# SidRama/Longitudinal-VAE

Hardware: AMD Instinct MI355X
Metric: ELBO-steps/sec (exact-KL L-VAE step, Health-MNIST N=4096 L=16) (higher is better)
Workload: dtype f16x3-split (fp32-equivalent)

## Files before the change

longitudinal-vae_amd/csrc/kl_hyper.hip:

```cpp
#include "blkinv.hpp"
#include "gram_tab.hpp"
#include "prof.hpp"

namespace lvae {

constexpr int kHbMaxBin = 4;
constexpr int kHbBins = 128;
constexpr int kHbBins2 = 4096;
constexpr int kHbRun = 64;
constexpr int kHbSmall = 16;
constexpr int kHbSmallest = 4;
constexpr int kHbNear = 4;
constexpr int kHbBlk = 4;
constexpr int kHbT = 64;
constexpr int kHbTP = 68;
constexpr int kHbNB = 24;
constexpr int kHbNQ = kHbNB / 4;
constexpr int kHbNearS = 2 * kHbBins2;
constexpr int kHbNearK = kHbNearS + kHbNear + 1;
constexpr int kHbA = kHbNearK + kHbNear;
constexpr int kHbTail = 2 * kHbNear + 1 + kHbBins;
constexpr int kHbPart = 2 * kHbBins2 + kHbTail;

struct HbDev {
  int on, nbin, big, nbins, nb2, nnear;
  int gmin[kTabMaxBits], grng[kTabMaxBits];
  int wmin[kTabMaxG], wrng[kTabMaxG];
  int bmask[kHbMaxBin], bgrp[kHbMaxBin], boff[kHbMaxBin], bn[kHbMaxBin], b2off[kHbMaxBin];
  int cbin[LVAE_MAX_COMP];
  int nslot[kHbNear];
};

typedef unsigned hb_u32x4 __attribute__((ext_vector_type(4)));

struct HbWs {
  HbDev* dev;
  uint8_t* pbin;
  int* rs;
  int* re;
  double* part;
  float* tab;
  hb_u32x4* rkey;
  double* hscr;
  double* nscr;
  size_t bytes;
  HbWs(char* base, int np_, int L) {
    size_t off = 0;
    auto take = [&](size_t b) {
      char* p = base ? base + off : nullptr;
      off += align256(b);
      return p;
    };
    dev = (HbDev*)take(sizeof(HbDev));
    pbin = (uint8_t*)take((size_t)kHbMaxBin * np_);
    rs = (int*)take((size_t)np_ * sizeof(int));
    re = (int*)take((size_t)np_ * sizeof(int));
    part = (double*)take((size_t)L * (np_ / kHbT) * kHbPart * sizeof(double));
    tab = (float*)take((size_t)L * kTabMaxBwdLds * sizeof(float));
    rkey = (hb_u32x4*)take((size_t)np_ * sizeof(hb_u32x4));
    hscr = (double*)take((size_t)L * (np_ / kHbT) * kHbBins * kHbT * sizeof(double));
    nscr = (double*)take((size_t)L * (np_ / kHbT) * kHbNB * 256 * sizeof(double));
    bytes = off;
  }
};
size_t kl_hyper_bytes(int np_, int L) { return HbWs(nullptr, np_, L).bytes; }
HbDev* kl_hyper_dev(void* base, int np_, int L) { return HbWs((char*)base, np_, L).dev; }

__global__ __launch_bounds__(1024) void hb_plan_kernel(GramTab tb, const double* __restrict__ x, int ldx, int n,
                                                       int np_, const int* __restrict__ covflag, HbWs ws, int enable) {
  __shared__ int lo[kTabMaxBits + kTabMaxG], hi[kTabMaxBits + kTabMaxG];
  __shared__ int fail;
  __shared__ HbDev d;
  const int tid = threadIdx.x, nd = tb.nbits + tb.ng;
  if (*covflag != 2) {
    if (tid == 0) ws.dev->on = 0;
    return;
  }
  if (tid < kTabMaxBits + kTabMaxG) {
    lo[tid] = INT_MAX;
    hi[tid] = INT_MIN;
  }
  if (tid == 0) fail = 0;
  __syncthreads();
  for (int q = 0; q < nd; ++q) {
    const int dim = q < tb.nbits ? tb.bdim[q] : tb.gdim[q - tb.nbits];
    if (dim < 0) continue;
    int mn = INT_MAX, mx = INT_MIN;
    for (int i = tid; i < n; i += 1024) {
      const int v = (int)x[(int64_t)i * ldx + dim];
      mn = min(mn, v);
      mx = max(mx, v);
    }
#pragma unroll
    for (int o = 32; o > 0; o >>= 1) {
      mn = min(mn, __shfl_xor(mn, o, 64));
      mx = max(mx, __shfl_xor(mx, o, 64));
    }
    if ((tid & 63) == 0) {
      atomicMin(&lo[q], mn);
      atomicMax(&hi[q], mx);
    }
  }
  __syncthreads();
  if (tid == 0) {
    HbDev p{};
    int f = 0;
    p.big = -1;
    for (int b = 0; b < tb.nbits; ++b) {
      p.gmin[b] = lo[b];
      p.grng[b] = hi[b] - lo[b] + 1;
      if (tb.bkind[b] == LVAE_CAT && p.grng[b] > kHbSmallest && (p.big < 0 || p.grng[b] > p.grng[p.big])) p.big = b;
    }
    for (int b = 0; b < tb.nbits; ++b)
      if (b != p.big && tb.bkind[b] == LVAE_CAT && p.grng[b] > kHbSmall) f = 1;
    for (int g = 0; g < tb.ng; ++g) {
      p.wmin[g] = tb.gdim[g] >= 0 ? lo[tb.nbits + g] : 0;
      p.wrng[g] = tb.gdim[g] >= 0 ? hi[tb.nbits + g] - lo[tb.nbits + g] + 1 : 1;
    }
    for (int r = 0; r < tb.n_comp; ++r) {
      p.cbin[r] = -1;
      if (p.big >= 0 && ((tb.cmask[r] >> p.big) & 1)) continue;
      const int grp = tb.ckind[r] >= 0 ? tb.cgrp[r] : -1;
      int g = 0;
      while (g < p.nbin && !(p.bmask[g] == tb.cmask[r] && p.bgrp[g] == grp)) ++g;
      if (g == p.nbin) {
        if (p.nbin == kHbMaxBin) {
          f = 1;
          break;
        }
        long long nb = grp >= 0 ? p.wrng[grp] : 1;
        for (int b = 0; b < tb.nbits; ++b)
          if ((tb.cmask[r] >> b) & 1) nb *= p.grng[b];
        if (nb > kHbBins) {
          f = 1;
          break;
        }
        p.bmask[g] = tb.cmask[r];
        p.bgrp[g] = grp;
        p.bn[g] = (int)nb;
        p.boff[g] = p.nbins;
        p.b2off[g] = p.nb2;
        p.nbins += (int)nb;
        p.nb2 += (int)(nb * nb);
        ++p.nbin;
      }
      p.cbin[r] = g;
    }
    if (p.nbins > kHbBins || p.nb2 > kHbBins2) f = 1;
    {
      int nblk = 0;
      for (int g = 0; g < p.nbin; ++g) nblk += (p.bn[g] + 31) / 32;
      if (nblk > kHbBlk) f = 1;
    }
    for (int k = 0; k < tb.pbeg[tb.ng] && !f; ++k)
      if (p.cbin[tb.pcomp[tb.porder[k]]] < 0) {
        if (p.nnear == kHbNear) f = 1;
        else p.nslot[p.nnear++] = k;
      }
    d = p;
    fail = f;
  }
  __syncthreads();
  const int bd = d.big >= 0 ? tb.bdim[d.big] : -1;
  int bad = 0;
  for (int i = tid; i < np_; i += 1024) {
    int s = -1, e = -1;
    if (bd >= 0 && i < n) {
      const double v = x[(int64_t)i * ldx + bd];
      if (i > 0 && x[(int64_t)(i - 1) * ldx + bd] > v) bad = 1;
      s = i;
      while (s > 0 && i - s < kHbRun && x[(int64_t)(s - 1) * ldx + bd] == v) --s;
      e = i + 1;
      while (e < n && e - i < kHbRun && x[(int64_t)e * ldx + bd] == v) ++e;
      if (e - s > kHbRun || (s > 0 && x[(int64_t)(s - 1) * ldx + bd] == v) || (e < n && x[(int64_t)e * ldx + bd] == v))
        bad = 1;
    }
    ws.rs[i] = s;
    ws.re[i] = e;
    hb_u32x4 key = {0u, 0u, 0u, 0u};
    if (i < n) {
      for (int b = 0; b < tb.nbits; ++b) {
        const int xv = (int)x[(int64_t)i * ldx + tb.bdim[b]], v = xv - d.gmin[b];
        if (b == d.big) continue;
        if (tb.bkind[b] == LVAE_CAT) {
          if (v < 0 || v > 63) bad = 1;
          key.x |= (unsigned)(v & 63) << (6 * b);
        } else {
          if (xv != 0 && xv != 1) bad = 1;
          key.w |= (unsigned)(xv == 1) << b;
        }
      }
      for (int g = 0; g < tb.ng; ++g) {
        if (tb.gdim[g] < 0) continue;
        const int v = (int)x[(int64_t)i * ldx + tb.gdim[g]] - d.wmin[g];
        if (v < 0 || v > 65535) bad = 1;
        const unsigned u = (unsigned)(v & 0xffff);
        if (g == 0) key.y |= u;
        else if (g == 1) key.y |= u << 16;
        else key.z |= u;
      }
    }
    ws.rkey[i] = key;
    for (int g = 0; g < kHbMaxBin; ++g) {
      int idx = 255;
      if (g < d.nbin && i < n) {
        idx = 0;
        for (int b = 0; b < tb.nbits; ++b)
          if ((d.bmask[g] >> b) & 1) idx = idx * d.grng[b] + ((int)x[(int64_t)i * ldx + tb.bdim[b]] - d.gmin[b]);
        if (d.bgrp[g] >= 0) idx = idx * d.wrng[d.bgrp[g]] + ((int)x[(int64_t)i * ldx + tb.gdim[d.bgrp[g]]] - d.wmin[d.bgrp[g]]);
      }
      ws.pbin[(size_t)g * np_ + i] = (uint8_t)idx;
    }
  }
  if (__any(bad) && (tid & 63) == 0) atomicOr(&fail, 1);
  __syncthreads();
  if (tid == 0) {
    HbDev p = d;
    p.on = (!fail && enable) ? 1 : 0;
    *ws.dev = p;
  }
}


__global__ __launch_bounds__(256) void hb_tab_kernel(GramTab tb, HbWs ws, const double* __restrict__ params) {
  __shared__ float sp[64];
  const int tid = threadIdx.x, l = blockIdx.y, e = blockIdx.x * 256 + tid;
  if (!ws.dev->on) return;
  if (tid < tb.n_params) sp[tid] = float(params[(int64_t)l * tb.n_params + tid]);
  __syncthreads();
  if (e < tb.pbeg[tb.ng] * (1 << tb.nbits) * kTabR) ws.tab[(int64_t)l * kTabMaxBwdLds + e] = tab_bwd_entry(tb, sp, e);
}

__device__ inline unsigned hb_pair_code(hb_u32x4 ki, hb_u32x4 kj, unsigned catbits, int ng) {
  const unsigned x = ki.x ^ kj.x, x1 = x | (x >> 1), x3 = x1 | (x1 >> 2), x5 = x3 | (x1 >> 4);
  const unsigned fail = (((x5 & 0x1041041u) * 0x108421u) >> 20) & 31u;
  unsigned c = (catbits & ~fail) | (ki.w & kj.w);
  const unsigned a0 = ki.y & 0xffffu, b0 = kj.y & 0xffffu, a1 = ki.y >> 16, b1 = kj.y >> 16;
  const unsigned a2 = ki.z & 0xffffu, b2 = kj.z & 0xffffu;
  const unsigned d0 = a0 > b0 ? a0 - b0 : b0 - a0, d1 = a1 > b1 ? a1 - b1 : b1 - a1, d2 = a2 > b2 ? a2 - b2 : b2 - a2;
  const unsigned cap = (unsigned)kTabD;
  c |= (d0 < cap ? d0 : cap) << 8;
  if (ng > 1) c |= (d1 < cap ? d1 : cap) << 16;
  if (ng > 2) c |= (d2 < cap ? d2 : cap) << 24;
  return c;
}

__device__ inline unsigned hb_catbits(const GramTab& tb) {
  unsigned m = 0;
#pragma unroll
  for (int b = 0; b < kTabMaxBits; ++b)
    if (b < tb.nbits && tb.bkind[b] == LVAE_CAT) m |= 1u << b;
  return m;
}

__device__ inline void hb_near_tables(const GramTab& tb, const HbDev& d, const float* __restrict__ gt, int tstride,
                                      float* __restrict__ tab, int* __restrict__ sgrp) {
  const int tid = threadIdx.x;
  if (tid < d.nnear) sgrp[tid] = tb.cgrp[tb.pcomp[tb.porder[d.nslot[tid]]]];
  for (int e = tid; e < d.nnear * tstride; e += blockDim.x) tab[e] = gt[d.nslot[e / tstride] * tstride + e % tstride];
}

__device__ inline float hb_near_d(const float* tab, int tk, unsigned code, int grp) {
  return tab[tk + (int)(code & 0xffu) * kTabR + (int)((code >> (8 * (grp + 1))) & 0xffu)];
}

__global__ __launch_bounds__(256) void hb_near_kernel(GramTab tb, HbWs ws, int n, int np_,
                                                      const float* __restrict__ Kinv, const double* __restrict__ alpha) {
  __shared__ HbDev d;
  __shared__ int sgrp[kHbNear];
  __shared__ double red[4][kHbNear];
  extern __shared__ float ntab[];
  const int tid = threadIdx.x, lane = tid & 63, w = tid >> 6, I = blockIdx.x, l = blockIdx.y, I0 = I * kHbT;
  if (tid == 0) d = *ws.dev;
  __syncthreads();
  if (!d.on) return;
  const int tstride = (1 << tb.nbits) * kTabR, nnear = d.nnear;
  hb_near_tables(tb, d, ws.tab + (int64_t)l * kTabMaxBwdLds, tstride, ntab, sgrp);
  __syncthreads();
  const float* K = Kinv + (int64_t)l * np_ * np_;
  const double* al = alpha + (int64_t)l * np_;
  const unsigned catbits = hb_catbits(tb);
  double acc[kHbNear];
#pragma unroll
  for (int k = 0; k < kHbNear; ++k) acc[k] = 0.0;
  if (d.big >= 0) {
    for (int e = tid; e < kHbT * kHbRun; e += 256) {
      const int i = I0 + e / kHbRun, jj = e % kHbRun;
      if (i >= n) continue;
      const int s = ws.rs[i], len = ws.re[i] - s;
      if (jj >= len) continue;
      const int j = s + jj;
      const unsigned c = hb_pair_code(ws.rkey[i], ws.rkey[j], catbits, tb.ng);
      const double val = 0.5 * ((double)K[(int64_t)i * np_ + j] - al[i] * al[j]);
#pragma unroll
      for (int k = 0; k < kHbNear; ++k)
        if (k < nnear) acc[k] += val * (double)hb_near_d(ntab, k * tstride, c, sgrp[k]);
    }
  }
#pragma unroll
  for (int k = 0; k < kHbNear; ++k) {
    const double sk = wave_sum(acc[k]);
    if (lane == 0) red[w][k] = sk;
  }
  __syncthreads();
  if (tid < kHbNear)
    ws.part[((int64_t)l * (np_ / kHbT) + I) * kHbPart + kHbNearK + tid] =
        ((red[0][tid] + red[1][tid]) + red[2][tid]) + red[3][tid];
}


#ifdef LVAE_HB_STAMP
#define HB_STAMP(t)                                                                   \
  do {                                                                                \
    __builtin_amdgcn_sched_barrier(0);                                                \
    asm volatile("s_memtime %0\n\ts_waitcnt lgkmcnt(0)" : "=s"(t)::"memory");       \
    __builtin_amdgcn_sched_barrier(0);                                                \
  } while (0)
#else
#define HB_STAMP(t) \
  do {              \
  } while (0)
#endif

typedef float hb_f32x2 __attribute__((ext_vector_type(2)));
typedef float hb_f32x4 __attribute__((ext_vector_type(4)));
typedef float hb_f32x16 __attribute__((ext_vector_type(16)));
typedef __bf16 hb_bf16x8 __attribute__((ext_vector_type(8)));
typedef __bf16 hb_bf16x2 __attribute__((ext_vector_type(2)));
constexpr int kHbSlabThreads = 256, kHbSlabWaves = kHbSlabThreads / 64;
#ifndef LVAE_HB_FOLD
#define LVAE_HB_FOLD 16
#endif
constexpr int kHbFold = LVAE_HB_FOLD;
#ifndef LVAE_HB_DEPTH
#define LVAE_HB_DEPTH 1
#endif
constexpr int kHbDepth = LVAE_HB_DEPTH;
static_assert(kHbDepth == 1 || kHbDepth == 2 || kHbDepth == 4, "nt = np / 64 is a multiple of 4");

struct HbPre {
  hb_f32x2 pk[8];
  int pbn;
  hb_f32x4 vr[2];
};

__device__ inline unsigned hb_pk_bf16(float a, float b) {
  const hb_bf16x2 v = {(__bf16)a, (__bf16)b};
  return __builtin_bit_cast(unsigned, v);
}
__device__ inline float hb_bf_lo(unsigned u) { return __uint_as_float(u << 16); }
__device__ inline float hb_bf_hi(unsigned u) { return __uint_as_float(u & 0xffff0000u); }

__device__ inline int hb_pl_off(int c, int k) { return c * 32 + ((k ^ ((c >> 1) & 7)) << 2); }

__device__ inline void hb_split8(const float* a, hb_u32x4& hi, hb_u32x4& mid, hb_u32x4& lo) {
#pragma unroll
  for (int k = 0; k < 4; ++k) {
    const float x0 = a[2 * k], x1 = a[2 * k + 1];
    const unsigned h = hb_pk_bf16(x0, x1);
    const float r0 = x0 - hb_bf_lo(h), r1 = x1 - hb_bf_hi(h);
    const unsigned m = hb_pk_bf16(r0, r1);
    const float s0 = r0 - hb_bf_lo(m), s1 = r1 - hb_bf_hi(m);
    hi[k] = h;
    mid[k] = m;
    lo[k] = hb_pk_bf16(s0, s1);
  }
}

__global__ __launch_bounds__(kHbSlabThreads, 2) void hb_slab_kernel(GramTab tb, HbWs ws, int n, int np_,
                                                                    const float* __restrict__ Kinv,
                                                                    const float* __restrict__ vv,
                                                                    const double* __restrict__ alpha) {
  __shared__ HbDev d;
  __shared__ __attribute__((aligned(16))) float Tc[2 * kHbT * kHbTP];
  __shared__ __attribute__((aligned(16))) unsigned Pw[3][kHbT * 32];
  __shared__ __attribute__((aligned(8))) uint8_t rbin[kHbMaxBin][kHbT];
  __shared__ uint8_t cbin[kHbMaxBin][kHbT];
  __shared__ float vs[kHbT];
  __shared__ double acol[kHbT];
  __shared__ hb_u32x4 ckey[2 * kHbT];
  __shared__ int rstart[kHbT];
  __shared__ unsigned long long runends;
  __shared__ int nblk, nspan;
  __shared__ uint8_t blist[kHbNB];
  __shared__ int8_t blkid[64];
  __shared__ int sgrp[kHbNear];
  __shared__ int sbg[kHbBlk], sbb[kHbBlk], nbk;
  __shared__ double red[kHbSlabWaves][kHbNear + 1];
  extern __shared__ float tab[];
  const int tid = threadIdx.x, lane = tid & 63, w = tid >> 6, J = blockIdx.x, l = blockIdx.y, J0 = J * kHbT;
  if (tid == 0) d = *ws.dev;
  __syncthreads();
  if (!d.on) return;
  const int tstride = (1 << tb.nbits) * kTabR;
  if (tid < kHbT) {
    vs[tid] = vv[(int64_t)l * np_ + J0 + tid];
    acol[tid] = alpha[(int64_t)l * np_ + J0 + tid];
  }
  for (int e = tid; e < d.nbin * kHbT; e += kHbSlabThreads)
    cbin[e / kHbT][e % kHbT] = ws.pbin[(size_t)(e / kHbT) * np_ + J0 + e % kHbT];
  hb_near_tables(tb, d, ws.tab + (int64_t)l * kTabMaxBwdLds, tstride, tab, sgrp);
  if (tid < 2 * kHbT) {
    const int c = J0 - kHbT + tid;
    ckey[tid] = c >= 0 ? ws.rkey[c] : hb_u32x4{0u, 0u, 0u, 0u};
  }
  if (w == 0) {
    const int c = J0 + lane;
    const bool isend = d.big >= 0 && c < n && ws.re[c] == c + 1;
    const int s0 = isend ? ws.rs[c] : c;
    rstart[lane] = s0;
    const int ba = (s0 - J0 + kHbT) >> 4, bz = (c - J0 + kHbT) >> 4;
    unsigned long long m = 0;
    if (isend)
      for (int bi = ba; bi <= bz; ++bi)
        for (int bj = ba; bj <= bi; ++bj) m |= 1ull << (bi * 8 + bj);
#pragma unroll
    for (int o = 32; o > 0; o >>= 1) {
      const unsigned lo = __shfl_xor((unsigned)m, o, 64), hi = __shfl_xor((unsigned)(m >> 32), o, 64);
      m |= ((unsigned long long)hi << 32) | lo;
    }
    const unsigned long long ends = __ballot(isend), sp = __ballot(isend && s0 < J0);
    if (lane == 0) {
      runends = ends;
      nspan = sp != 0;
      int t = 0;
      for (int b = 0; b < 64; ++b) {
        blkid[b] = -1;
        if (((m >> b) & 1ull) && t < kHbNB) {
          blkid[b] = (int8_t)t;
          blist[t++] = (uint8_t)b;
        }
      }
      nblk = t;
    }
  }
  if (tid == 0) {
    int t = 0;
    for (int g = 0; g < d.nbin; ++g)
      for (int bb = 0; bb * 32 < d.bn[g] && t < kHbBlk; ++bb, ++t) {
        sbg[t] = g;
        sbb[t] = bb;
      }
    nbk = t;
  }
  __syncthreads();
  const float* K = Kinv + (int64_t)l * np_ * np_;
  const int nbin = d.nbin, nnear = d.nnear, nitem = 2 * nbk, nbl = nblk, span = nspan;
  const unsigned catbits = hb_catbits(tb);
  const int cb = w & 1, hh = lane >> 5, col = 32 * cb + (lane & 31);
  const int i0 = w, i1 = w + kHbSlabWaves;
  const bool it0 = i0 < nitem, it1 = i1 < nitem;
  int g0 = 0, b00 = 0, g1 = 0, b01 = 0;
  if (it0) {
    g0 = sbg[i0 >> 1];
    b00 = 32 * sbb[i0 >> 1];
  }
  if (it1) {
    g1 = sbg[i1 >> 1];
    b01 = 32 * sbb[i1 >> 1];
  }
  hb_f32x16 acc0 = {}, acc1 = {};
  double* Hs = ws.hscr + ((int64_t)l * (np_ / kHbT) + J) * kHbBins * kHbT;
  double* Ns = ws.nscr + ((int64_t)l * (np_ / kHbT) + J) * kHbNB * 256;
  const int li = lane & 15, lk = lane >> 4;
  bi_f32x4 nac[kHbNQ];
#pragma unroll
  for (int q = 0; q < kHbNQ; ++q) nac[q] = bi_f32x4{0.f, 0.f, 0.f, 0.f};
  double tS = 0.0;
  const int cp = tid & 31, i8 = tid >> 5;
  const float v0 = vs[2 * cp], v1 = vs[2 * cp + 1], r0 = sqrtf(v0), r1 = sqrtf(v1);
  const int nt = np_ / kHbT;

  auto fetch = [&](int I, HbPre& p) {
    const int I0 = I * kHbT;
#pragma unroll
    for (int u = 0; u < 8; ++u)
      p.pk[u] = __builtin_nontemporal_load(
          reinterpret_cast<const hb_f32x2*>(K + (int64_t)(I0 + 8 * i8 + u) * np_ + J0 + 2 * cp));
    p.pbn = (int)ws.pbin[(size_t)(w < nbin ? w : 0) * np_ + I0 + lane];
    const float* vr = vv + (int64_t)l * np_ + I0 + 8 * i8;
    p.vr[0] = *reinterpret_cast<const hb_f32x4*>(vr);
    p.vr[1] = *reinterpret_cast<const hb_f32x4*>(vr + 4);
  };

  auto fold = [&](hb_f32x16& acc, int g, int b0, bool first) {
    const int nb = d.bn[g];
    double* hc = Hs + (int64_t)d.boff[g] * kHbT + col;
#pragma unroll
    for (int e = 0; e < 16; ++e) {
      const int b = b0 + (e & 3) + 8 * (e >> 2) + 4 * hh;
      if (b < nb) {
        if (first) hc[b * kHbT] = (double)acc[e];
        else unsafeAtomicAdd(hc + b * kHbT, (double)acc[e]);
      }
      acc[e] = 0.f;
    }
  };

  auto body = [&](int I, HbPre& p) {
    const int I0 = I * kHbT;
    const bool fold_now = (I & (kHbFold - 1)) == kHbFold - 1 || I == nt - 1, fold_first = I < kHbFold;
    {
      float ts = 0.f;
#pragma unroll
      for (int u = 0; u < 8; ++u) {
        const float s0 = p.pk[u][0] * r0, s1 = p.pk[u][1] * r1;
        ts += s0 * s0 + s1 * s1;
      }
      tS += (double)ts;
#pragma unroll
      for (int c = 0; c < 2; ++c) {
        float a[8];
#pragma unroll
        for (int u = 0; u < 8; ++u) a[u] = p.pk[u][c];
        hb_u32x4 hi, mid, lo;
        hb_split8(a, hi, mid, lo);
        const int off = hb_pl_off(2 * cp + c, i8);
        *reinterpret_cast<hb_u32x4*>(&Pw[0][off]) = hi;
        *reinterpret_cast<hb_u32x4*>(&Pw[1][off]) = mid;
        *reinterpret_cast<hb_u32x4*>(&Pw[2][off]) = lo;
      }
    }
    if (w < nbin) rbin[w][lane] = (uint8_t)p.pbn;
    if (nbl > 0) {
      float sr[8];
#pragma unroll
      for (int u = 0; u < 8; ++u) sr[u] = sqrtf(p.vr[u >> 2][u & 3]);
#pragma unroll
      for (int c = 0; c < 2; ++c) {
        float* dst = &Tc[(kHbT + 2 * cp + c) * kHbTP + 8 * i8];
        *reinterpret_cast<hb_f32x4*>(dst) = hb_f32x4{p.pk[0][c] * sr[0], p.pk[1][c] * sr[1], p.pk[2][c] * sr[2],
                                                     p.pk[3][c] * sr[3]};
        *reinterpret_cast<hb_f32x4*>(dst + 4) = hb_f32x4{p.pk[4][c] * sr[4], p.pk[5][c] * sr[5],
                                                         p.pk[6][c] * sr[6], p.pk[7][c] * sr[7]};
      }
      if (span) {
        hb_f32x2 q[8];
#pragma unroll
        for (int u = 0; u < 8; ++u)
          q[u] = *reinterpret_cast<const hb_f32x2*>(K + (int64_t)(I0 + 8 * i8 + u) * np_ + J0 - kHbT + 2 * cp);
#pragma unroll
        for (int c = 0; c < 2; ++c) {
          float* dst = &Tc[(2 * cp + c) * kHbTP + 8 * i8];
          *reinterpret_cast<hb_f32x4*>(dst) = hb_f32x4{q[0][c] * sr[0], q[1][c] * sr[1], q[2][c] * sr[2],
                                                       q[3][c] * sr[3]};
          *reinterpret_cast<hb_f32x4*>(dst + 4) = hb_f32x4{q[4][c] * sr[4], q[5][c] * sr[5], q[6][c] * sr[6],
                                                           q[7][c] * sr[7]};
        }
      }
    }
    __syncthreads();
    fetch(I + kHbDepth < nt ? I + kHbDepth : nt - 1, p);
    if (it0) {
      auto onehot = [&](int g, int b0, int ks) {
        const unsigned mybin = (unsigned)(b0 + (lane & 31));
        const uint2 rb = *reinterpret_cast<const uint2*>(&rbin[g][16 * ks + 8 * hh]);
        hb_u32x4 a;
#pragma unroll
        for (int k = 0; k < 4; ++k) {
          const unsigned wd = k < 2 ? rb.x : rb.y, sh = 16 * (k & 1);
          const unsigned lo_ = ((wd >> sh) & 0xffu) == mybin ? 0x3f80u : 0u;
          const unsigned hi_ = ((wd >> (sh + 8)) & 0xffu) == mybin ? 0x3f800000u : 0u;
          a[k] = lo_ | hi_;
        }
        return __builtin_bit_cast(hb_bf16x8, a);
      };
#pragma unroll
      for (int ks = 0; ks < 4; ++ks) {
        const hb_bf16x8 bh = *reinterpret_cast<const hb_bf16x8*>(&Pw[0][hb_pl_off(col, 2 * ks + hh)]);
        const hb_bf16x8 bm = *reinterpret_cast<const hb_bf16x8*>(&Pw[1][hb_pl_off(col, 2 * ks + hh)]);
        const hb_bf16x8 bl = *reinterpret_cast<const hb_bf16x8*>(&Pw[2][hb_pl_off(col, 2 * ks + hh)]);
        const hb_bf16x8 a0 = onehot(g0, b00, ks);
        acc0 = __builtin_amdgcn_mfma_f32_32x32x16_bf16(a0, bl, acc0, 0, 0, 0);
        acc0 = __builtin_amdgcn_mfma_f32_32x32x16_bf16(a0, bm, acc0, 0, 0, 0);
        acc0 = __builtin_amdgcn_mfma_f32_32x32x16_bf16(a0, bh, acc0, 0, 0, 0);
        if (it1) {
          const hb_bf16x8 a1 = onehot(g1, b01, ks);
          acc1 = __builtin_amdgcn_mfma_f32_32x32x16_bf16(a1, bl, acc1, 0, 0, 0);
          acc1 = __builtin_amdgcn_mfma_f32_32x32x16_bf16(a1, bm, acc1, 0, 0, 0);
          acc1 = __builtin_amdgcn_mfma_f32_32x32x16_bf16(a1, bh, acc1, 0, 0, 0);
        }
      }
      if (fold_now) {
        fold(acc0, g0, b00, fold_first);
        if (it1) fold(acc1, g1, b01, fold_first);
      }
    }
#pragma unroll
    for (int q = 0; q < kHbNQ; ++q) {
      const int t = w + kHbSlabWaves * q;
      if (t < nbl) {
        const int bb = blist[t], bi = bb >> 3, bj = bb & 7;
        const float* pa = &Tc[(16 * bi + li) * kHbTP + 16 * lk];
        const float* pb = &Tc[(16 * bj + li) * kHbTP + 16 * lk];
        hb_f32x4 a4[4], b4[4];
#pragma unroll
        for (int s4 = 0; s4 < 4; ++s4) {
          a4[s4] = *reinterpret_cast<const hb_f32x4*>(pa + 4 * s4);
          b4[s4] = *reinterpret_cast<const hb_f32x4*>(pb + 4 * s4);
        }
        bi_f32x4 x0 = {0.f, 0.f, 0.f, 0.f}, x1 = {0.f, 0.f, 0.f, 0.f};
#pragma unroll
        for (int s4 = 0; s4 < 4; ++s4) {
          x0 = __builtin_amdgcn_mfma_f32_16x16x4f32(a4[s4][0], b4[s4][0], x0, 0, 0, 0);
          x1 = __builtin_amdgcn_mfma_f32_16x16x4f32(a4[s4][1], b4[s4][1], x1, 0, 0, 0);
          x0 = __builtin_amdgcn_mfma_f32_16x16x4f32(a4[s4][2], b4[s4][2], x0, 0, 0, 0);
          x1 = __builtin_amdgcn_mfma_f32_16x16x4f32(a4[s4][3], b4[s4][3], x1, 0, 0, 0);
        }
        nac[q] += x0 + x1;
        if (fold_now) {
          double* nb = Ns + t * 256 + (4 * lk) * 16 + li;
#pragma unroll
          for (int e = 0; e < 4; ++e) {
            if (fold_first) nb[e * 16] = (double)nac[q][e];
            else unsafeAtomicAdd(nb + e * 16, (double)nac[q][e]);
          }
          nac[q] = bi_f32x4{0.f, 0.f, 0.f, 0.f};
        }
      }
    }
    __syncthreads();
  };

  HbPre pre[kHbDepth];
#pragma unroll
  for (int u = 0; u < kHbDepth; ++u) fetch(u, pre[u]);
  for (int I = 0; I < nt; I += kHbDepth) {
#pragma unroll
    for (int u = 0; u < kHbDepth; ++u) body(I + u, pre[u]);
  }
  __builtin_amdgcn_s_waitcnt(0);
  __threadfence_block();
  __syncthreads();
  double* Qs = reinterpret_cast<double*>(&Tc[0]);
  for (int e = tid; e < d.nb2; e += kHbSlabThreads) Qs[e] = 0.0;
  __syncthreads();
  double* out = ws.part + ((int64_t)l * nt + J) * kHbPart;
  for (int tb2 = tid; tb2 < d.nbins; tb2 += kHbSlabThreads) {
    int g = 0;
    while (g + 1 < nbin && tb2 >= d.boff[g + 1]) ++g;
    const int b = tb2 - d.boff[g], nb = d.bn[g];
    double* qrow = Qs + d.b2off[g] + b * nb;
    const double* hr = Hs + (int64_t)tb2 * kHbT;
    double as = 0.0;
    for (int m = 0; m < kHbT; ++m) {
      const int bc = cbin[g][m];
      if (bc != 255) qrow[bc] += hr[m];
      if (bc == b) as += acol[m];
    }
    out[kHbA + tb2] = as;
  }
  __syncthreads();
  for (int e = tid; e < d.nb2; e += kHbSlabThreads) out[kHbBins2 + e] = Qs[e];
  for (int g = 0; g < nbin; ++g) {
    const int nb = d.bn[g], nb16 = (nb + 15) >> 4;
    for (int item = w; item < nb16 * nb16; item += kHbSlabWaves) {
      const int bi = item / nb16, bj = item % nb16, li = lane & 15, lk = lane >> 4;
      const int ba = 16 * bi + li, bb = 16 * bj + li;
      const double* ha = Hs + (int64_t)(d.boff[g] + (ba < nb ? ba : 0)) * kHbT;
      const double* hb = Hs + (int64_t)(d.boff[g] + (bb < nb ? bb : 0)) * kHbT;
      bi_f64x4 acc = {0.0, 0.0, 0.0, 0.0};
#pragma unroll 4
      for (int s4 = 0; s4 < kHbT; s4 += 4) {
        const int m = s4 + lk;
        const double a = ba < nb ? ha[m] * (double)vs[m] : 0.0;
        const double b = bb < nb ? hb[m] : 0.0;
        acc = __builtin_amdgcn_mfma_f64_16x16x4f64(a, b, acc, 0, 0, 0);
      }
#pragma unroll
      for (int q = 0; q < 4; ++q) {
        const int r = 16 * bi + lk + 4 * q, c = 16 * bj + li;
        if (r < nb && c < nb) out[d.b2off[g] + r * nb + c] = acc[q];
      }
    }
  }
  double nacc[kHbNear];
#pragma unroll
  for (int k = 0; k < kHbNear; ++k) nacc[k] = 0.0;
  for (unsigned long long rm = runends; rm; rm &= rm - 1) {
    const int e = __builtin_ctzll(rm), s0 = rstart[e], len = e + 1 - (s0 - J0);
    for (int pq = tid; pq < len * len; pq += kHbSlabThreads) {
      const int wi = s0 - J0 + kHbT + pq / len, wj = s0 - J0 + kHbT + pq % len;
      const int lo_ = min(wi, wj), hi_ = max(wi, wj);
      const int t = blkid[((hi_ >> 4) << 3) | (lo_ >> 4)];
      const double sv = t >= 0 ? Ns[t * 256 + (hi_ & 15) * 16 + (lo_ & 15)] : 0.0;
      const unsigned c = hb_pair_code(ckey[wi], ckey[wj], catbits, tb.ng);
      const int cb8 = (int)(c & 0xffu) * kTabR;
#pragma unroll
      for (int k2 = 0; k2 < kHbNear; ++k2) {
        if (k2 >= nnear) break;
        const int g = sgrp[k2];
        nacc[k2] += sv * (double)tab[k2 * tstride + cb8 + (int)((c >> (8 * (g + 1))) & 0xffu)];
      }
    }
  }
#pragma unroll
  for (int k = 0; k < kHbNear; ++k) {
    const double sk = wave_sum(nacc[k]);
    if (lane == 0) red[w][k] = sk;
  }
  {
    const double st = wave_sum(tS);
    if (lane == 0) red[w][kHbNear] = st;
  }
  __syncthreads();
  if (tid <= kHbNear) {
    double t = 0.0;
#pragma unroll
    for (int u = 0; u < kHbSlabWaves; ++u) t += red[u][tid];
    out[kHbNearS + tid] = t;
  }
}

constexpr int kNoiseSlotHb = 64, kBwdSlotsHb = 65;

__global__ __launch_bounds__(256) void hb_sum_kernel(HbWs ws, int np_) {
  const int i = blockIdx.x * 256 + threadIdx.x, l = blockIdx.y, nt = np_ / kHbT, nb2 = ws.dev->nb2;
  if (!ws.dev->on || i >= 2 * nb2 + kHbTail) return;
  const int e = i < nb2 ? i : i < 2 * nb2 ? kHbBins2 + i - nb2 : 2 * kHbBins2 + i - 2 * nb2;
  double* pl = ws.part + (int64_t)l * nt * kHbPart + e;
  double s = 0.0;
#pragma unroll 16
  for (int J = 0; J < nt; ++J) s += pl[(int64_t)J * kHbPart];
  pl[0] = s;
}

__global__ __launch_bounds__(256) void hb_final_kernel(GramTab tb, HbWs ws, int n, int np_,
                                                       const double* __restrict__ alpha,
                                                       const double* __restrict__ kdiag, double* __restrict__ part,
                                                       int G) {
  __shared__ HbDev d;
  __shared__ double Gb[kHbBins2];
  __shared__ double raw[kBwdSlotsHb];
  __shared__ double red[4];
  __shared__ double nz;
  extern __shared__ float ftab[];
  const int tid = threadIdx.x, lane = tid & 63, w = tid >> 6, l = blockIdx.x, nt = np_ / kHbT;
  if (tid == 0) d = *ws.dev;
  __syncthreads();
  if (!d.on) return;
  if (tid < kBwdSlotsHb) raw[tid] = 0.0;
  const double* al = alpha + (int64_t)l * np_;
  const double* pl = ws.part + (int64_t)l * nt * kHbPart;
  {
    const float* gt = ws.tab + (int64_t)l * kTabMaxBwdLds;
    for (int e = tid; e < tb.pbeg[tb.ng] * (1 << tb.nbits) * kTabR; e += 256) ftab[e] = gt[e];
  }
  for (int e = tid; e < d.nb2; e += 256) {
    int g = 0;
    while (g + 1 < d.nbin && e >= d.b2off[g + 1]) ++g;
    const int nb = d.bn[g], b = (e - d.b2off[g]) / nb, bc = (e - d.b2off[g]) % nb;
    const double m = pl[e], q = pl[kHbBins2 + e];
    Gb[e] = 0.5 * (q - m - pl[kHbA + d.boff[g] + b] * pl[kHbA + d.boff[g] + bc]);
  }
  {
    double s = 0.0;
    for (int i = tid; i < n; i += 256) s += kdiag[(int64_t)l * np_ + i] - al[i] * al[i];
    s = wave_sum(s);
    if (lane == 0) red[w] = s;
  }
  __syncthreads();
  if (tid == 0) {
    nz = 0.5 * ((((red[0] + red[1]) + red[2]) + red[3]) - pl[kHbNearS + kHbNear]);
    for (int k = 0; k < d.nnear; ++k)
      raw[tb.porder[d.nslot[k]]] = -0.5 * pl[kHbNearS + k] + pl[kHbNearK + k];
  }
  const int tstride = (1 << tb.nbits) * kTabR;
  for (int k = 0; k < tb.pbeg[tb.ng]; ++k) {
    const int p = tb.porder[k], r = tb.pcomp[p], g = d.cbin[r];
    if (g < 0) continue;
    const int nb = d.bn[g], grp = d.bgrp[g], W = grp >= 0 ? d.wrng[grp] : 1;
    double s = 0.0;
    for (int e = tid; e < nb * nb; e += 256) {
      int b = e / nb, bc = e % nb;
      const int w1 = b % W, w2 = bc % W;
      b /= W;
      bc /= W;
      int bits = 0;
#pragma unroll
      for (int q = kTabMaxBits - 1; q >= 0; --q) {
        if (q >= tb.nbits || !((d.bmask[g] >> q) & 1)) continue;
        const int v1 = b % d.grng[q] + d.gmin[q], v2 = bc % d.grng[q] + d.gmin[q];
        b /= d.grng[q];
        bc /= d.grng[q];
        const bool pass = tb.bkind[q] == LVAE_CAT ? v1 == v2 : v1 + v2 == 2;
        bits += pass ? (kTabR << q) : 0;
      }
      s += Gb[d.b2off[g] + e] * (double)ftab[k * tstride + bits + abs(w1 - w2)];
    }
    s = wave_sum(s);
    __syncthreads();
    if (lane == 0) red[w] = s;
    __syncthreads();
    if (tid == 0) raw[p] = ((red[0] + red[1]) + red[2]) + red[3];
  }
  __syncthreads();
  if (tid == 0) raw[kNoiseSlotHb] = nz;
  __syncthreads();
  for (int e = tid; e < kBwdSlotsHb * G; e += 256) {
    const int slot = e / G, gg = e % G;
    part[((int64_t)l * kBwdSlotsHb + slot) * G + gg] = gg == 0 ? raw[slot] : 0.0;
  }
}

static int hb_enabled() {
  const char* v = getenv("LVAE_KL_HYPER");
  return !v || atoi(v) != 0;
}

static size_t hb_slab_lds(const GramTab& tb) {
  static size_t stat = 0;
  if (!stat) {
    hipFuncAttributes a;
    if (hipFuncGetAttributes(&a, reinterpret_cast<const void*>(&hb_slab_kernel)) != hipSuccess) return 0;
    stat = a.sharedSizeBytes;
  }
  const int ns = tb.pbeg[tb.ng] < kHbNear ? tb.pbeg[tb.ng] : kHbNear;
  const size_t dyn = (size_t)ns * (1 << tb.nbits) * kTabR * sizeof(float);
  return stat + dyn <= 160 * 1024 ? (dyn ? dyn : 4) : 0;
}

static bool hb_host_ok(const lvae_kernel_spec* spec, GramTab& tb) {
  return gram_tab_build(spec, tb) && hb_enabled() && hb_slab_lds(tb) > 0;
}

int kl_hyper_plan(const lvae_kernel_spec* spec, const double* x, int ldx, int n, int np_, int L, void* wsbase,
                  const int* covflag, hipStream_t st) {
  HbWs ws((char*)wsbase, np_, L);
  GramTab tb;
  if (!hb_host_ok(spec, tb)) {
    if (zero_async(ws.dev, sizeof(HbDev), st) != 0) return LVAE_ERR_LAUNCH;
    return 0;
  }
  hb_plan_kernel<<<1, 1024, 0, st>>>(tb, x, ldx, n, np_, covflag, ws, 1);
  LVAE_CHECK_LAUNCH();
  return 0;
}

int kl_hyper_bwd(const lvae_kernel_spec* spec, const double* x, int ldx, int n, int np_, int L, const double* params,
                 const float* Kinv, const float* v, const double* alpha, const double* kdiag, void* wsbase, double* part,
                 int G, hipStream_t st) {
  (void)x;
  (void)ldx;
  HbWs ws((char*)wsbase, np_, L);
  GramTab tb;
  if (!gram_tab_build(spec, tb) || hb_slab_lds(tb) == 0) return 0;
  const size_t tabb = (size_t)tb.pbeg[tb.ng] * (1 << tb.nbits) * kTabR * sizeof(float);
  const size_t sdyn = hb_slab_lds(tb), ndyn = sdyn;
  const int nt = np_ / kHbT;
  hb_tab_kernel<<<dim3((unsigned)((tabb / sizeof(float) + 255) / 256), L), 256, 0, st>>>(tb, ws, params);
  hb_near_kernel<<<dim3(nt, L), 256, ndyn, st>>>(tb, ws, n, np_, Kinv, alpha);
  {
    ProfScope ps(LVAE_PH_HB_SLAB, st);
    hb_slab_kernel<<<dim3(nt, L), kHbSlabThreads, sdyn, st>>>(tb, ws, n, np_, Kinv, v, alpha);
  }
  hb_sum_kernel<<<dim3((2 * kHbBins2 + kHbTail + 255) / 256, L), 256, 0, st>>>(ws, np_);
  hb_final_kernel<<<L, 256, tabb, st>>>(tb, ws, n, np_, alpha, kdiag, part, G);
  LVAE_CHECK_LAUNCH();
  return 0;
}

}

extern "C" int lvae_kl_closed_hyper_state(int n, int L, const void* workspace, int32_t* on, void* stream) {
  if (n <= 0) return -1;
  if (L <= 0) return -2;
  if (!workspace) return -3;
  if (!on) return -4;
  size_t kl_hyper_offset_in_kl_ws(int np_, int L);
  const int np_ = (n + 255) / 256 * 256;
  const char* hb = (const char*)workspace + kl_hyper_offset_in_kl_ws(np_, L);
  const lvae::HbWs ws(const_cast<char*>(hb), np_, L);
  if (lvae::copy_words_async(on, &ws.dev->on, sizeof(int32_t), (hipStream_t)stream) != 0) return LVAE_ERR_LAUNCH;
  return 0;
}
```

Measured before the change: 122.7.

## Split slab kernel across row chunks with separate reduction/finish kernel

The slab kernel is now launched with a third grid dimension that splits the row-tile loop into chunks of kHbFold tiles. Each chunk writes its fp32 partial histogram, near-block and trace accumulators to per-chunk scratch, replacing the in-loop double-precision atomic folds. A new finish kernel sums the chunk partials in double and then runs the Q-row, near-term and output epilogue that used to sit at the end of the slab kernel. This exposes more blocks to fill the GPU, at the cost of extra scratch memory traffic, one more launch, and fp32 rather than double storage of each chunk's partial sums.

```diff
diff --git a/longitudinal-vae_amd/csrc/kl_hyper.hip b/longitudinal-vae_amd/csrc/kl_hyper.hip
--- a/longitudinal-vae_amd/csrc/kl_hyper.hip
+++ b/longitudinal-vae_amd/csrc/kl_hyper.hip
@@ -13,6 +13,7 @@
 constexpr int kHbNear = 4;
 constexpr int kHbBlk = 4;
 constexpr int kHbT = 64;
+constexpr int kHbFold = 16;
 constexpr int kHbTP = 68;
 constexpr int kHbNB = 24;
 constexpr int kHbNQ = kHbNB / 4;
@@ -33,6 +34,8 @@
 
 typedef unsigned hb_u32x4 __attribute__((ext_vector_type(4)));
 
+inline int hb_chunks(int np_) { return (np_ / kHbT + kHbFold - 1) / kHbFold; }
+
 struct HbWs {
   HbDev* dev;
   uint8_t* pbin;
@@ -41,8 +44,11 @@
   double* part;
   float* tab;
   hb_u32x4* rkey;
-  double* hscr;
-  double* nscr;
+  float* hscr;
+  float* nscr;
+  double* tscr;
+  double* hsum;
+  double* nsum;
   size_t bytes;
   HbWs(char* base, int np_, int L) {
     size_t off = 0;
@@ -58,8 +64,12 @@
     part = (double*)take((size_t)L * (np_ / kHbT) * kHbPart * sizeof(double));
     tab = (float*)take((size_t)L * kTabMaxBwdLds * sizeof(float));
     rkey = (hb_u32x4*)take((size_t)np_ * sizeof(hb_u32x4));
-    hscr = (double*)take((size_t)L * (np_ / kHbT) * kHbBins * kHbT * sizeof(double));
-    nscr = (double*)take((size_t)L * (np_ / kHbT) * kHbNB * 256 * sizeof(double));
+    const size_t chunks = (size_t)L * (np_ / kHbT) * hb_chunks(np_);
+    hscr = (float*)take(chunks * kHbBins * kHbT * sizeof(float));
+    nscr = (float*)take(chunks * kHbNB * 256 * sizeof(float));
+    tscr = (double*)take(chunks * sizeof(double));
+    hsum = (double*)take((size_t)L * (np_ / kHbT) * kHbBins * kHbT * sizeof(double));
+    nsum = (double*)take((size_t)L * (np_ / kHbT) * kHbNB * 256 * sizeof(double));
     bytes = off;
   }
 };
@@ -309,34 +319,19 @@
 }
 
 
-#ifdef LVAE_HB_STAMP
-#define HB_STAMP(t)                                                                   \
-  do {                                                                                \
-    __builtin_amdgcn_sched_barrier(0);                                                \
-    asm volatile("s_memtime %0\n\ts_waitcnt lgkmcnt(0)" : "=s"(t)::"memory");       \
-    __builtin_amdgcn_sched_barrier(0);                                                \
-  } while (0)
-#else
-#define HB_STAMP(t) \
-  do {              \
-  } while (0)
-#endif
-
 typedef float hb_f32x2 __attribute__((ext_vector_type(2)));
 typedef float hb_f32x4 __attribute__((ext_vector_type(4)));
 typedef float hb_f32x16 __attribute__((ext_vector_type(16)));
+typedef double hb_f64x2 __attribute__((ext_vector_type(2)));
 typedef __bf16 hb_bf16x8 __attribute__((ext_vector_type(8)));
 typedef __bf16 hb_bf16x2 __attribute__((ext_vector_type(2)));
 constexpr int kHbSlabThreads = 256, kHbSlabWaves = kHbSlabThreads / 64;
-#ifndef LVAE_HB_FOLD
-#define LVAE_HB_FOLD 16
-#endif
-constexpr int kHbFold = LVAE_HB_FOLD;
 #ifndef LVAE_HB_DEPTH
 #define LVAE_HB_DEPTH 1
 #endif
 constexpr int kHbDepth = LVAE_HB_DEPTH;
-static_assert(kHbDepth == 1 || kHbDepth == 2 || kHbDepth == 4, "nt = np / 64 is a multiple of 4");
+static_assert(kHbDepth == 1 || kHbDepth == 2 || kHbDepth == 4, "a chunk's tile count is a multiple of 4");
+static_assert(kHbFold % 4 == 0, "nt = np / 64 is a multiple of 4, so every chunk's tile count is one too");
 
 struct HbPre {
   hb_f32x2 pk[8];
@@ -367,74 +362,57 @@
   }
 }
 
+__device__ inline void hb_near_window(const HbDev& d, const HbWs& ws, int n, int J0, int lane, int* nblk, int* nspan,
+                                      uint8_t* blist, int* rstart, unsigned long long* runends, int8_t* blkid) {
+  const int c = J0 + lane;
+  const bool isend = d.big >= 0 && c < n && ws.re[c] == c + 1;
+  const int s0 = isend ? ws.rs[c] : c;
+  if (rstart) rstart[lane] = s0;
+  const int ba = (s0 - J0 + kHbT) >> 4, bz = (c - J0 + kHbT) >> 4;
+  unsigned long long m = 0;
+  if (isend)
+    for (int bi = ba; bi <= bz; ++bi)
+      for (int bj = ba; bj <= bi; ++bj) m |= 1ull << (bi * 8 + bj);
+#pragma unroll
+  for (int o = 32; o > 0; o >>= 1) {
+    const unsigned lo = __shfl_xor((unsigned)m, o, 64), hi = __shfl_xor((unsigned)(m >> 32), o, 64);
+    m |= ((unsigned long long)hi << 32) | lo;
+  }
+  const unsigned long long ends = __ballot(isend), sp = __ballot(isend && s0 < J0);
+  if (lane == 0) {
+    if (runends) *runends = ends;
+    *nspan = sp != 0;
+    int t = 0;
+    for (int b = 0; b < 64; ++b) {
+      if (blkid) blkid[b] = -1;
+      if (((m >> b) & 1ull) && t < kHbNB) {
+        if (blkid) blkid[b] = (int8_t)t;
+        blist[t++] = (uint8_t)b;
+      }
+    }
+    *nblk = t;
+  }
+}
+
 __global__ __launch_bounds__(kHbSlabThreads, 2) void hb_slab_kernel(GramTab tb, HbWs ws, int n, int np_,
                                                                     const float* __restrict__ Kinv,
-                                                                    const float* __restrict__ vv,
-                                                                    const double* __restrict__ alpha) {
+                                                                    const float* __restrict__ vv) {
   __shared__ HbDev d;
   __shared__ __attribute__((aligned(16))) float Tc[2 * kHbT * kHbTP];
   __shared__ __attribute__((aligned(16))) unsigned Pw[3][kHbT * 32];
   __shared__ __attribute__((aligned(8))) uint8_t rbin[kHbMaxBin][kHbT];
-  __shared__ uint8_t cbin[kHbMaxBin][kHbT];
   __shared__ float vs[kHbT];
-  __shared__ double acol[kHbT];
-  __shared__ hb_u32x4 ckey[2 * kHbT];
-  __shared__ int rstart[kHbT];
-  __shared__ unsigned long long runends;
   __shared__ int nblk, nspan;
   __shared__ uint8_t blist[kHbNB];
-  __shared__ int8_t blkid[64];
-  __shared__ int sgrp[kHbNear];
   __shared__ int sbg[kHbBlk], sbb[kHbBlk], nbk;
-  __shared__ double red[kHbSlabWaves][kHbNear + 1];
-  extern __shared__ float tab[];
+  __shared__ double red[kHbSlabWaves];
   const int tid = threadIdx.x, lane = tid & 63, w = tid >> 6, J = blockIdx.x, l = blockIdx.y, J0 = J * kHbT;
   if (tid == 0) d = *ws.dev;
   __syncthreads();
   if (!d.on) return;
-  const int tstride = (1 << tb.nbits) * kTabR;
-  if (tid < kHbT) {
-    vs[tid] = vv[(int64_t)l * np_ + J0 + tid];
-    acol[tid] = alpha[(int64_t)l * np_ + J0 + tid];
-  }
-  for (int e = tid; e < d.nbin * kHbT; e += kHbSlabThreads)
-    cbin[e / kHbT][e % kHbT] = ws.pbin[(size_t)(e / kHbT) * np_ + J0 + e % kHbT];
-  hb_near_tables(tb, d, ws.tab + (int64_t)l * kTabMaxBwdLds, tstride, tab, sgrp);
-  if (tid < 2 * kHbT) {
-    const int c = J0 - kHbT + tid;
-    ckey[tid] = c >= 0 ? ws.rkey[c] : hb_u32x4{0u, 0u, 0u, 0u};
-  }
-  if (w == 0) {
-    const int c = J0 + lane;
-    const bool isend = d.big >= 0 && c < n && ws.re[c] == c + 1;
-    const int s0 = isend ? ws.rs[c] : c;
-    rstart[lane] = s0;
-    const int ba = (s0 - J0 + kHbT) >> 4, bz = (c - J0 + kHbT) >> 4;
-    unsigned long long m = 0;
-    if (isend)
-      for (int bi = ba; bi <= bz; ++bi)
-        for (int bj = ba; bj <= bi; ++bj) m |= 1ull << (bi * 8 + bj);
-#pragma unroll
-    for (int o = 32; o > 0; o >>= 1) {
-      const unsigned lo = __shfl_xor((unsigned)m, o, 64), hi = __shfl_xor((unsigned)(m >> 32), o, 64);
-      m |= ((unsigned long long)hi << 32) | lo;
-    }
-    const unsigned long long ends = __ballot(isend), sp = __ballot(isend && s0 < J0);
-    if (lane == 0) {
-      runends = ends;
-      nspan = sp != 0;
-      int t = 0;
-      for (int b = 0; b < 64; ++b) {
-        blkid[b] = -1;
-        if (((m >> b) & 1ull) && t < kHbNB) {
-          blkid[b] = (int8_t)t;
-          blist[t++] = (uint8_t)b;
-        }
-      }
-      nblk = t;
-    }
-  }
-  if (tid == 0) {
+  if (tid < kHbT) vs[tid] = vv[(int64_t)l * np_ + J0 + tid];
+  if (w == 0) hb_near_window(d, ws, n, J0, lane, &nblk, &nspan, blist, nullptr, nullptr, nullptr);
+  if (tid == 64) {
     int t = 0;
     for (int g = 0; g < d.nbin; ++g)
       for (int bb = 0; bb * 32 < d.bn[g] && t < kHbBlk; ++bb, ++t) {
@@ -445,8 +423,7 @@
   }
   __syncthreads();
   const float* K = Kinv + (int64_t)l * np_ * np_;
-  const int nbin = d.nbin, nnear = d.nnear, nitem = 2 * nbk, nbl = nblk, span = nspan;
-  const unsigned catbits = hb_catbits(tb);
+  const int nbin = d.nbin, nitem = 2 * nbk, nbl = nblk, span = nspan;
   const int cb = w & 1, hh = lane >> 5, col = 32 * cb + (lane & 31);
   const int i0 = w, i1 = w + kHbSlabWaves;
   const bool it0 = i0 < nitem, it1 = i1 < nitem;
@@ -460,8 +437,6 @@
     b01 = 32 * sbb[i1 >> 1];
   }
   hb_f32x16 acc0 = {}, acc1 = {};
-  double* Hs = ws.hscr + ((int64_t)l * (np_ / kHbT) + J) * kHbBins * kHbT;
-  double* Ns = ws.nscr + ((int64_t)l * (np_ / kHbT) + J) * kHbNB * 256;
   const int li = lane & 15, lk = lane >> 4;
   bi_f32x4 nac[kHbNQ];
 #pragma unroll
@@ -469,7 +444,8 @@
   double tS = 0.0;
   const int cp = tid & 31, i8 = tid >> 5;
   const float v0 = vs[2 * cp], v1 = vs[2 * cp + 1], r0 = sqrtf(v0), r1 = sqrtf(v1);
-  const int nt = np_ / kHbT;
+  const int nt = np_ / kHbT, R = (int)gridDim.z, r = blockIdx.z;
+  const int Ia = r * kHbFold, Iz = min(Ia + kHbFold, nt);
 
   auto fetch = [&](int I, HbPre& p) {
     const int I0 = I * kHbT;
@@ -483,23 +459,8 @@
     p.vr[1] = *reinterpret_cast<const hb_f32x4*>(vr + 4);
   };
 
-  auto fold = [&](hb_f32x16& acc, int g, int b0, bool first) {
-    const int nb = d.bn[g];
-    double* hc = Hs + (int64_t)d.boff[g] * kHbT + col;
-#pragma unroll
-    for (int e = 0; e < 16; ++e) {
-      const int b = b0 + (e & 3) + 8 * (e >> 2) + 4 * hh;
-      if (b < nb) {
-        if (first) hc[b * kHbT] = (double)acc[e];
-        else unsafeAtomicAdd(hc + b * kHbT, (double)acc[e]);
-      }
-      acc[e] = 0.f;
-    }
-  };
-
   auto body = [&](int I, HbPre& p) {
     const int I0 = I * kHbT;
-    const bool fold_now = (I & (kHbFold - 1)) == kHbFold - 1 || I == nt - 1, fold_first = I < kHbFold;
     {
       float ts = 0.f;
 #pragma unroll
@@ -550,7 +511,7 @@
       }
     }
     __syncthreads();
-    fetch(I + kHbDepth < nt ? I + kHbDepth : nt - 1, p);
+    fetch(I + kHbDepth < Iz ? I + kHbDepth : Iz - 1, p);
     if (it0) {
       auto onehot = [&](int g, int b0, int ks) {
         const unsigned mybin = (unsigned)(b0 + (lane & 31));
@@ -581,10 +542,6 @@
           acc1 = __builtin_amdgcn_mfma_f32_32x32x16_bf16(a1, bh, acc1, 0, 0, 0);
         }
       }
-      if (fold_now) {
-        fold(acc0, g0, b00, fold_first);
-        if (it1) fold(acc1, g1, b01, fold_first);
-      }
     }
 #pragma unroll
     for (int q = 0; q < kHbNQ; ++q) {
@@ -593,30 +550,17 @@
         const int bb = blist[t], bi = bb >> 3, bj = bb & 7;
         const float* pa = &Tc[(16 * bi + li) * kHbTP + 16 * lk];
         const float* pb = &Tc[(16 * bj + li) * kHbTP + 16 * lk];
-        hb_f32x4 a4[4], b4[4];
+        bi_f32x4 x0 = {0.f, 0.f, 0.f, 0.f}, x1 = {0.f, 0.f, 0.f, 0.f};
 #pragma unroll
         for (int s4 = 0; s4 < 4; ++s4) {
-          a4[s4] = *reinterpret_cast<const hb_f32x4*>(pa + 4 * s4);
-          b4[s4] = *reinterpret_cast<const hb_f32x4*>(pb + 4 * s4);
-        }
-        bi_f32x4 x0 = {0.f, 0.f, 0.f, 0.f}, x1 = {0.f, 0.f, 0.f, 0.f};
-#pragma unroll
-        for (int s4 = 0; s4 < 4; ++s4) {
-          x0 = __builtin_amdgcn_mfma_f32_16x16x4f32(a4[s4][0], b4[s4][0], x0, 0, 0, 0);
-          x1 = __builtin_amdgcn_mfma_f32_16x16x4f32(a4[s4][1], b4[s4][1], x1, 0, 0, 0);
-          x0 = __builtin_amdgcn_mfma_f32_16x16x4f32(a4[s4][2], b4[s4][2], x0, 0, 0, 0);
-          x1 = __builtin_amdgcn_mfma_f32_16x16x4f32(a4[s4][3], b4[s4][3], x1, 0, 0, 0);
+          const hb_f32x4 a4 = *reinterpret_cast<const hb_f32x4*>(pa + 4 * s4);
+          const hb_f32x4 b4 = *reinterpret_cast<const hb_f32x4*>(pb + 4 * s4);
+          x0 = __builtin_amdgcn_mfma_f32_16x16x4f32(a4[0], b4[0], x0, 0, 0, 0);
+          x1 = __builtin_amdgcn_mfma_f32_16x16x4f32(a4[1], b4[1], x1, 0, 0, 0);
+          x0 = __builtin_amdgcn_mfma_f32_16x16x4f32(a4[2], b4[2], x0, 0, 0, 0);
+          x1 = __builtin_amdgcn_mfma_f32_16x16x4f32(a4[3], b4[3], x1, 0, 0, 0);
         }
         nac[q] += x0 + x1;
-        if (fold_now) {
-          double* nb = Ns + t * 256 + (4 * lk) * 16 + li;
-#pragma unroll
-          for (int e = 0; e < 4; ++e) {
-            if (fold_first) nb[e * 16] = (double)nac[q][e];
-            else unsafeAtomicAdd(nb + e * 16, (double)nac[q][e]);
-          }
-          nac[q] = bi_f32x4{0.f, 0.f, 0.f, 0.f};
-        }
       }
     }
     __syncthreads();
@@ -624,16 +568,124 @@
 
   HbPre pre[kHbDepth];
 #pragma unroll
-  for (int u = 0; u < kHbDepth; ++u) fetch(u, pre[u]);
-  for (int I = 0; I < nt; I += kHbDepth) {
+  for (int u = 0; u < kHbDepth; ++u) fetch(Ia + u, pre[u]);
+  for (int I = Ia; I < Iz; I += kHbDepth) {
 #pragma unroll
     for (int u = 0; u < kHbDepth; ++u) body(I + u, pre[u]);
   }
-  __builtin_amdgcn_s_waitcnt(0);
+  const int64_t pr = ((int64_t)l * nt + J) * R + r;
+  if (it0) {
+    float* Hs = ws.hscr + pr * (kHbBins * kHbT);
+    auto store = [&](const hb_f32x16& acc, int g, int b0) {
+      const int nb = d.bn[g];
+      float* hc = Hs + (int64_t)d.boff[g] * kHbT + col;
+#pragma unroll
+      for (int e = 0; e < 16; ++e) {
+        const int b = b0 + (e & 3) + 8 * (e >> 2) + 4 * hh;
+        if (b < nb) hc[b * kHbT] = acc[e];
+      }
+    };
+    store(acc0, g0, b00);
+    if (it1) store(acc1, g1, b01);
+  }
+  {
+    float* Ns = ws.nscr + pr * (kHbNB * 256);
+#pragma unroll
+    for (int q = 0; q < kHbNQ; ++q) {
+      const int t = w + kHbSlabWaves * q;
+      if (t < nbl) {
+        float* nb = Ns + t * 256 + (4 * lk) * 16 + li;
+#pragma unroll
+        for (int e = 0; e < 4; ++e) nb[e * 16] = nac[q][e];
+      }
+    }
+  }
+  {
+    const double st = wave_sum(tS);
+    if (lane == 0) red[w] = st;
+    __syncthreads();
+    if (tid == 0) ws.tscr[pr] = ((red[0] + red[1]) + red[2]) + red[3];
+  }
+}
+
+__global__ __launch_bounds__(kHbSlabThreads, 4) void hb_slab_fin_kernel(GramTab tb, HbWs ws, int n, int np_, int R,
+                                                                     const float* __restrict__ vv,
+                                                                     const double* __restrict__ alpha) {
+  __shared__ HbDev d;
+  __shared__ double Qs[kHbBins2];
+  __shared__ uint8_t cbin[kHbMaxBin][kHbT];
+  __shared__ float vs[kHbT];
+  __shared__ double acol[kHbT];
+  __shared__ hb_u32x4 ckey[2 * kHbT];
+  __shared__ int rstart[kHbT];
+  __shared__ unsigned long long runends;
+  __shared__ int nblk, nspan;
+  __shared__ uint8_t blist[kHbNB];
+  __shared__ int8_t blkid[64];
+  __shared__ int sgrp[kHbNear];
+  __shared__ double red[kHbSlabWaves][kHbNear];
+  extern __shared__ float tab[];
+  const int tid = threadIdx.x, lane = tid & 63, w = tid >> 6, J = blockIdx.x, l = blockIdx.y, J0 = J * kHbT;
+  if (tid == 0) d = *ws.dev;
+  __syncthreads();
+  if (!d.on) return;
+  const int tstride = (1 << tb.nbits) * kTabR, nt = np_ / kHbT;
+  if (tid < kHbT) {
+    vs[tid] = vv[(int64_t)l * np_ + J0 + tid];
+    acol[tid] = alpha[(int64_t)l * np_ + J0 + tid];
+  }
+  for (int e = tid; e < d.nbin * kHbT; e += kHbSlabThreads)
+    cbin[e / kHbT][e % kHbT] = ws.pbin[(size_t)(e / kHbT) * np_ + J0 + e % kHbT];
+  hb_near_tables(tb, d, ws.tab + (int64_t)l * kTabMaxBwdLds, tstride, tab, sgrp);
+  if (tid < 2 * kHbT) {
+    const int c = J0 - kHbT + tid;
+    ckey[tid] = c >= 0 ? ws.rkey[c] : hb_u32x4{0u, 0u, 0u, 0u};
+  }
+  if (w == 0) hb_near_window(d, ws, n, J0, lane, &nblk, &nspan, blist, rstart, &runends, blkid);
+  for (int e = tid; e < d.nb2; e += kHbSlabThreads) Qs[e] = 0.0;
+  __syncthreads();
+  const int nbin = d.nbin, nnear = d.nnear;
+  const unsigned catbits = hb_catbits(tb);
+  const int64_t p0 = ((int64_t)l * nt + J) * R;
+  double tS = ws.tscr[p0];
+  for (int r = 1; r < R; ++r) tS += ws.tscr[p0 + r];
+  double* Hs = ws.hsum + ((int64_t)l * nt + J) * (kHbBins * kHbT);
+  double* Ns = ws.nsum + ((int64_t)l * nt + J) * (kHbNB * 256);
+  {
+    constexpr int kPer = kHbBins * kHbT / kHbSlabThreads;
+    const float* __restrict__ Hp = ws.hscr + p0 * (kHbBins * kHbT);
+    const int lim = d.nbins * kHbT;
+    double hv[kPer];
+#pragma unroll
+    for (int i = 0; i < kPer; ++i)
+      hv[i] = tid + kHbSlabThreads * i < lim ? (double)Hp[tid + kHbSlabThreads * i] : 0.0;
+    for (int r = 1; r < R; ++r) {
+      const float* __restrict__ Hr = Hp + (int64_t)r * (kHbBins * kHbT);
+#pragma unroll
+      for (int i = 0; i < kPer; ++i)
+        if (tid + kHbSlabThreads * i < lim) hv[i] += (double)Hr[tid + kHbSlabThreads * i];
+    }
+#pragma unroll
+    for (int i = 0; i < kPer; ++i)
+      if (tid + kHbSlabThreads * i < lim) Hs[tid + kHbSlabThreads * i] = hv[i];
+  }
+  {
+    const float* __restrict__ Np = ws.nscr + p0 * (kHbNB * 256);
+    const int lim = nblk * 256;
+    double nv[kHbNB];
+#pragma unroll
+    for (int i = 0; i < kHbNB; ++i) nv[i] = 256 * i < lim ? (double)Np[tid + 256 * i] : 0.0;
+    for (int r = 1; r < R; ++r) {
+      const float* __restrict__ Nr = Np + (int64_t)r * (kHbNB * 256);
+#pragma unroll
+      for (int i = 0; i < kHbNB; ++i)
+        if (256 * i < lim) nv[i] += (double)Nr[tid + 256 * i];
+    }
+#pragma unroll
+    for (int i = 0; i < kHbNB; ++i)
+      if (256 * i < lim) Ns[tid + 256 * i] = nv[i];
+  }
   __threadfence_block();
-  __syncthreads();
-  double* Qs = reinterpret_cast<double*>(&Tc[0]);
-  for (int e = tid; e < d.nb2; e += kHbSlabThreads) Qs[e] = 0.0;
   __syncthreads();
   double* out = ws.part + ((int64_t)l * nt + J) * kHbPart;
   for (int tb2 = tid; tb2 < d.nbins; tb2 += kHbSlabThreads) {
@@ -641,12 +693,18 @@
     while (g + 1 < nbin && tb2 >= d.boff[g + 1]) ++g;
     const int b = tb2 - d.boff[g], nb = d.bn[g];
     double* qrow = Qs + d.b2off[g] + b * nb;
-    const double* hr = Hs + (int64_t)tb2 * kHbT;
     double as = 0.0;
-    for (int m = 0; m < kHbT; ++m) {
-      const int bc = cbin[g][m];
-      if (bc != 255) qrow[bc] += hr[m];
-      if (bc == b) as += acol[m];
+#pragma unroll 1
+    for (int m0 = 0; m0 < kHbT; m0 += 32) {
+      hb_f64x2 hr[16];
+#pragma unroll
+      for (int m = 0; m < 16; ++m) hr[m] = reinterpret_cast<const hb_f64x2*>(Hs + (int64_t)tb2 * kHbT + m0)[m];
+#pragma unroll
+      for (int m = 0; m < 32; ++m) {
+        const int bc = cbin[g][m0 + m];
+        if (bc != 255) qrow[bc] += hr[m >> 1][m & 1];
+        if (bc == b) as += acol[m0 + m];
+      }
     }
     out[kHbA + tb2] = as;
   }
@@ -660,7 +718,7 @@
       const double* ha = Hs + (int64_t)(d.boff[g] + (ba < nb ? ba : 0)) * kHbT;
       const double* hb = Hs + (int64_t)(d.boff[g] + (bb < nb ? bb : 0)) * kHbT;
       bi_f64x4 acc = {0.0, 0.0, 0.0, 0.0};
-#pragma unroll 4
+#pragma unroll
       for (int s4 = 0; s4 < kHbT; s4 += 4) {
         const int m = s4 + lk;
         const double a = ba < nb ? ha[m] * (double)vs[m] : 0.0;
@@ -699,17 +757,14 @@
     const double sk = wave_sum(nacc[k]);
     if (lane == 0) red[w][k] = sk;
   }
-  {
-    const double st = wave_sum(tS);
-    if (lane == 0) red[w][kHbNear] = st;
-  }
-  __syncthreads();
-  if (tid <= kHbNear) {
+  __syncthreads();
+  if (tid < kHbNear) {
     double t = 0.0;
 #pragma unroll
     for (int u = 0; u < kHbSlabWaves; ++u) t += red[u][tid];
     out[kHbNearS + tid] = t;
   }
+  if (tid == kHbNear) out[kHbNearS + kHbNear] = tS;
 }
 
 constexpr int kNoiseSlotHb = 64, kBwdSlotsHb = 65;
@@ -812,7 +867,7 @@
   static size_t stat = 0;
   if (!stat) {
     hipFuncAttributes a;
-    if (hipFuncGetAttributes(&a, reinterpret_cast<const void*>(&hb_slab_kernel)) != hipSuccess) return 0;
+    if (hipFuncGetAttributes(&a, reinterpret_cast<const void*>(&hb_slab_fin_kernel)) != hipSuccess) return 0;
     stat = a.sharedSizeBytes;
   }
   const int ns = tb.pbeg[tb.ng] < kHbNear ? tb.pbeg[tb.ng] : kHbNear;
@@ -847,13 +902,14 @@
   if (!gram_tab_build(spec, tb) || hb_slab_lds(tb) == 0) return 0;
   const size_t tabb = (size_t)tb.pbeg[tb.ng] * (1 << tb.nbits) * kTabR * sizeof(float);
   const size_t sdyn = hb_slab_lds(tb), ndyn = sdyn;
-  const int nt = np_ / kHbT;
+  const int nt = np_ / kHbT, R = hb_chunks(np_);
   hb_tab_kernel<<<dim3((unsigned)((tabb / sizeof(float) + 255) / 256), L), 256, 0, st>>>(tb, ws, params);
   hb_near_kernel<<<dim3(nt, L), 256, ndyn, st>>>(tb, ws, n, np_, Kinv, alpha);
   {
     ProfScope ps(LVAE_PH_HB_SLAB, st);
-    hb_slab_kernel<<<dim3(nt, L), kHbSlabThreads, sdyn, st>>>(tb, ws, n, np_, Kinv, v, alpha);
-  }
+    hb_slab_kernel<<<dim3(nt, L, R), kHbSlabThreads, 0, st>>>(tb, ws, n, np_, Kinv, v);
+  }
+  hb_slab_fin_kernel<<<dim3(nt, L), kHbSlabThreads, sdyn, st>>>(tb, ws, n, np_, R, v, alpha);
   hb_sum_kernel<<<dim3((2 * kHbBins2 + kHbTail + 255) / 256, L), 256, 0, st>>>(ws, np_);
   hb_final_kernel<<<L, 256, tabb, st>>>(tb, ws, n, np_, alpha, kdiag, part, G);
   LVAE_CHECK_LAUNCH();
```

Result: no change. 122.1 (-0.4%).
